# 4ment/physher

Measured on NVIDIA B200. Metric: lnL+gradient throughput (site patterns x tree nodes per second), higher is better.
Workload: dtype f64

## Files before the change

physher_b200/csrc/phb_nuc4.cu:

```cuda
#include "phb_ctx.cuh"

#include <math.h>
#include <stdlib.h>
#include <string.h>

#define NUC4_CHUNK PHBC_WALK_CHUNK
#define NUC4_NT 256
#ifndef NUC4_L2PF
#define NUC4_L2PF 1
#endif

struct Nuc4Params {
	int T, N, C, P, PB, root;
	int n_post, n_pre, nslots, ntiles;
	int include_root_freqs, compat;
	int nbatch, phases;
	long long mats_stride;
	int post_first_tips, pre_first_tips;
	double threshold;
	const uint8_t *tip_codes;
	const double *weights;
	const double *props;
	const phbc_post_op *post_ops;
	const phbc_pre_op *pre_ops;
	const double *post_mats;
	const double *pre_mats;
	double *lower;
	double *gacc;
	double *gstat;
	double *cta_lnl;
	double *pattern_lnl;
	double freqs[4];
	double fq[4];
	double wroot[4];
	double FQ[16];
	double FQ2[16];
	const double *rates;
	double *hacc;
};

__device__ __forceinline__ void matvec_smem(const double *__restrict__ M, const double (&x)[4], double (&y)[4]) {
	const double2 *M2 = reinterpret_cast<const double2 *>(M);
#pragma unroll
	for (int i = 0; i < 4; i++) {
		const double2 a = M2[2 * i], b = M2[2 * i + 1];
		y[i] = fma(a.x, x[0], fma(a.y, x[1], fma(b.x, x[2], b.y * x[3])));
	}
}

__device__ __forceinline__ void tip_message(const double *__restrict__ M, unsigned code, double (&y)[4]) {
	if (__all_sync(0xffffffffu, code < 4u)) {
#pragma unroll
		for (int i = 0; i < 4; i++) y[i] = M[4 * i + code];
	} else {
		double x[4];
#pragma unroll
		for (int j = 0; j < 4; j++) x[j] = (code < 4u ? code == (unsigned)j : ((code >> j) & 1u)) ? 1.0 : 0.0;
		matvec_smem(M, x, y);
		if (code == 4u) y[0] = y[1] = y[2] = y[3] = 1.0;
	}
}

#define NUC4_SLOT_BYTES (2 * NUC4_NT * 16)
#define NUC4_ROW_BYTES (NUC4_NT * 32)

__device__ __forceinline__ void cell_load(const unsigned char *cell, double (&x)[4]) {
	const double2 lo = *reinterpret_cast<const double2 *>(cell);
	const double2 hi = *reinterpret_cast<const double2 *>(cell + NUC4_NT * 16);
	x[0] = lo.x, x[1] = lo.y, x[2] = hi.x, x[3] = hi.y;
}
__device__ __forceinline__ void cell_store(unsigned char *cell, const double (&x)[4]) {
	*reinterpret_cast<double2 *>(cell) = make_double2(x[0], x[1]);
	*reinterpret_cast<double2 *>(cell + NUC4_NT * 16) = make_double2(x[2], x[3]);
}
__device__ __forceinline__ void row_load(const unsigned char *cell, double (&x)[4]) {
	const double2 lo = __ldcs(reinterpret_cast<const double2 *>(cell));
	const double2 hi = __ldcs(reinterpret_cast<const double2 *>(cell + NUC4_NT * 16));
	x[0] = lo.x, x[1] = lo.y, x[2] = hi.x, x[3] = hi.y;
}
__device__ __forceinline__ void row_store(unsigned char *cell, const double (&x)[4]) {
	__stcs(reinterpret_cast<double2 *>(cell), make_double2(x[0], x[1]));
	__stcs(reinterpret_cast<double2 *>(cell + NUC4_NT * 16), make_double2(x[2], x[3]));
}

struct Nuc4Stage {
	uint32_t desc_off, mat_off, code_off, bytes;
};
__host__ __device__ constexpr Nuc4Stage nuc4_stage_layout(int C, int PB) {
	return Nuc4Stage{64u, (uint32_t)(64 + NUC4_CHUNK * 48), (uint32_t)(64 + NUC4_CHUNK * 48 + NUC4_CHUNK * 3 * C * 128),
	                 (uint32_t)((64 + NUC4_CHUNK * 48 + NUC4_CHUNK * 3 * C * 128 + 2 * NUC4_CHUNK * PB + 127) & ~127)};
}

__device__ __forceinline__ double butterfly4(double v0, double v1, double v2, double v3, int lane) {
	const bool h16 = lane & 16, h8 = lane & 8;
	const double r01 = (h16 ? v1 : v0) + __shfl_xor_sync(0xffffffffu, h16 ? v0 : v1, 16);
	const double r23 = (h16 ? v3 : v2) + __shfl_xor_sync(0xffffffffu, h16 ? v2 : v3, 16);
	double r = (h8 ? r23 : r01) + __shfl_xor_sync(0xffffffffu, h8 ? r01 : r23, 8);
	r += __shfl_xor_sync(0xffffffffu, r, 4);
	r += __shfl_xor_sync(0xffffffffu, r, 2);
	r += __shfl_xor_sync(0xffffffffu, r, 1);
	return r;
}
__device__ __forceinline__ double butterfly2(double v0, double v1, int lane) {
	const bool h16 = lane & 16;
	double r = (h16 ? v1 : v0) + __shfl_xor_sync(0xffffffffu, h16 ? v0 : v1, 16);
	r += __shfl_xor_sync(0xffffffffu, r, 8);
	r += __shfl_xor_sync(0xffffffffu, r, 4);
	r += __shfl_xor_sync(0xffffffffu, r, 2);
	r += __shfl_xor_sync(0xffffffffu, r, 1);
	return r;
}

__device__ __forceinline__ void tip_vector(unsigned code, double (&x)[4]) {
#pragma unroll
	for (int j = 0; j < 4; j++) x[j] = (code < 4u ? code == (unsigned)j : (code == 4u || ((code >> j) & 1u))) ? 1.0 : 0.0;
}

template <int PPT>
__device__ __forceinline__ void gstat_add(const double (&t)[PPT][4], const double (&x)[PPT][4], double *row, int lane) {
	double v[16];
#pragma unroll
	for (int i = 0; i < 4; i++)
#pragma unroll
		for (int j = 0; j < 4; j++) {
			double a = t[0][i] * x[0][j];
#pragma unroll
			for (int u = 1; u < PPT; u++) a = fma(t[u][i], x[u][j], a);
			v[4 * i + j] = a;
		}
#pragma unroll
	for (int w = 8, off = 16; w >= 1; w >>= 1, off >>= 1) {
		const bool h = lane & off;
#pragma unroll
		for (int k = 0; k < w; k++) {
			const double keep = h ? v[w + k] : v[k], send = h ? v[k] : v[w + k];
			v[k] = keep + __shfl_xor_sync(0xffffffffu, send, off);
		}
	}
	v[0] += __shfl_xor_sync(0xffffffffu, v[0], 1);
	if (!(lane & 1)) red_add_f64(row + (lane >> 1), v[0]);
}

template <int PPT>
__device__ __forceinline__ void matvec_smem_n(const double *__restrict__ M, const double (&x)[PPT][4], double (&y)[PPT][4]) {
	const double2 *M2 = reinterpret_cast<const double2 *>(M);
#pragma unroll
	for (int i = 0; i < 4; i++) {
		const double2 a = M2[2 * i], b = M2[2 * i + 1];
#pragma unroll
		for (int u = 0; u < PPT; u++) y[u][i] = fma(a.x, x[u][0], fma(a.y, x[u][1], fma(b.x, x[u][2], b.y * x[u][3])));
	}
}

template <int C, bool SCALE, int GRAD, int PPT>
__global__ void __launch_bounds__(NUC4_NT / PPT, GRAD == 3 ? (PPT == 1 ? 1 : 2) : 3) k_nuc4_walk(const Nuc4Params prm) {
	extern __shared__ __align__(128) unsigned char smem_raw[];
	constexpr int PB = NUC4_NT / C;
	constexpr int NTHR = NUC4_NT / PPT;
	constexpr int PBT = PB / PPT;
	static_assert(PBT % 32 == 0 || PPT == 1, "a warp must not mix categories");
	static_assert(GRAD != 3 || !SCALE, "the Hessian walk is unscaled (rescaled evaluations take the resident-partials route)");
	constexpr bool RECOMP = GRAD == 1 && !SCALE;
	const int tid = threadIdx.x, lane = tid & 31, warp = tid >> 5;
	const int c = tid / PBT, pl0 = tid - c * PBT;
	const int cell0 = c * PB + pl0;
	constexpr Nuc4Stage lay = nuc4_stage_layout(C, PB);
	uint64_t *bars = reinterpret_cast<uint64_t *>(smem_raw);
	unsigned char *stage0 = smem_raw;
	unsigned char *slot_cell = stage0 + 2 * lay.bytes + cell0 * 16;
	double *xch = reinterpret_cast<double *>(stage0 + 2 * lay.bytes + (size_t)prm.nslots * NUC4_SLOT_BYTES);
	double *invLw = xch + (SCALE ? (GRAD == 2 ? 5 : 4) : (GRAD == 3 ? 2 : 1)) * C * PB;
	double *sfslot = invLw + PB;
	const uint32_t my_mat = lay.mat_off + c * 128;
	const uint32_t my_code = lay.code_off + pl0;

	if (tid == 0) {
		mbar_init(&bars[0], 1);
		mbar_init(&bars[1], 1);
		asm volatile("fence.mbarrier_init.release.cluster;" ::: "memory");
	}
	__syncthreads();

	uint32_t loads = 0;
	const double prop_c = (C == 1) ? 1.0 : prm.props[c];
	double cta_lnl = 0.0;
	unsigned char *row_cell = GRAD ? reinterpret_cast<unsigned char *>(prm.lower) + (size_t)blockIdx.x * prm.n_post * NUC4_ROW_BYTES + cell0 * 16 : nullptr;
	double *my_gacc = nullptr;
	double *my_gstat = GRAD == 2 ? prm.gstat + ((size_t)blockIdx.x * (NTHR / 32) + warp) * prm.N * 16 : nullptr;
	double *my_hacc = GRAD == 3 ? prm.hacc + ((size_t)blockIdx.x * (NTHR / 32) + warp) * prm.N : nullptr;
	const double rate_c = GRAD == 3 ? prm.rates[c] : 0.0;

	constexpr int PF_LPR = PPT * 2 * 4;
	const int pf_row = (lane / PF_LPR) & 1, pf_q = lane % PF_LPR;
	const bool pf_on = GRAD && lane < 2 * PF_LPR;
	const unsigned char *pf_base = GRAD ? row_cell - lane * 16 + ((pf_q >> 3) * PBT) * 16 + ((pf_q >> 2) & 1) * (NUC4_NT * 16) + (pf_q & 3) * 128 : nullptr;

	const long long nitems = (long long)prm.ntiles * prm.nbatch;
	const bool strided = prm.nbatch == 1;
	const int item0 = strided ? (int)blockIdx.x : (int)(blockIdx.x * nitems / gridDim.x);
	const int item1 = strided ? (int)nitems : (int)((blockIdx.x + 1) * nitems / gridDim.x);
	const int item_step = strided ? (int)gridDim.x : 1;
	const int b_first = strided ? 0 : item0 / prm.ntiles;
	int cur_b = -1;
	auto flush_lnl = [&](int b) {
		if (lane == 0) prm.cta_lnl[((size_t)blockIdx.x * prm.phases + (b - b_first)) * (NTHR / 32) + warp] = (c == 0) ? cta_lnl : 0.0;
	};

	for (int item = item0; item < item1; item += item_step) {
		const int bsmp = item / prm.ntiles, tile = item - bsmp * prm.ntiles;
		if (bsmp != cur_b) {
			if (cur_b >= 0) flush_lnl(cur_b);
			cur_b = bsmp;
			cta_lnl = 0.0;
			if (GRAD) my_gacc = prm.gacc + (((size_t)blockIdx.x * prm.phases + (bsmp - b_first)) * (NTHR / 32) + warp) * prm.N;
		}
		const uint8_t *tile_codes_post = prm.tip_codes + (size_t)tile * prm.T * PB;
		const uint8_t *tile_codes_pre = prm.tip_codes + ((size_t)prm.ntiles + tile) * prm.T * PB;

		double out[PPT][4];
// ... 35 lines not shown
					double sf_in[PPT];
#pragma unroll
					for (int u = 0; u < PPT; u++) sf_in[u] = 0.0;
					if (kind == 0) {
#pragma unroll
						for (int u = 0; u < PPT; u++) {
							tip_message(MA, cds[a_idx * PB + u * PBT], ma[u]);
							tip_message(MB, cds[b_idx * PB + u * PBT], out[u]);
						}
					} else {
						if (SCALE) {
#pragma unroll
							for (int u = 0; u < PPT; u++) sf_in[u] = sf_acc[u];
						}
						if (kind == 1) {
#pragma unroll
							for (int u = 0; u < PPT; u++) tip_message(MA, cds[a_idx * PB + u * PBT], ma[u]);
						} else {
#pragma unroll
							for (int u = 0; u < PPT; u++) {
								cell_load(slot_cell + a_idx * NUC4_SLOT_BYTES + u * PBT * 16, ma[u]);
								if (SCALE) sf_in[u] += sfslot[a_idx * NUC4_NT + cell0 + u * PBT];
							}
						}
					}
#pragma unroll
					for (int u = 0; u < PPT; u++)
#pragma unroll
						for (int i = 0; i < 4; i++) lw[u][i] = ma[u][i] * out[u][i];
					if (SCALE) {
						double *mx = xch + ((first + j) & 1) * C * PB;
#pragma unroll
						for (int u = 0; u < PPT; u++) mx[cell0 + u * PBT] = fmax(fmax(lw[u][0], lw[u][1]), fmax(lw[u][2], lw[u][3]));
						__syncthreads();
#pragma unroll
						for (int u = 0; u < PPT; u++) {
							const int pl = pl0 + u * PBT;
							double m = mx[pl];
							for (int cc = 1; cc < C; cc++) m = fmax(m, mx[cc * PB + pl]);
							double sf = 0.0;
							if (m < prm.threshold) {
#pragma unroll
								for (int i = 0; i < 4; i++) lw[u][i] /= m;
								sf = log(m);
							}
							sf_acc[u] = sf + sf_in[u];
							if (dst_slot >= 0) sfslot[dst_slot * NUC4_NT + cell0 + u * PBT] = sf_acc[u];
						}
					}
					matvec_smem_n<PPT>(MN, lw, out);
#pragma unroll
					for (int u = 0; u < PPT; u++) {
						if (dst_slot >= 0) cell_store(slot_cell + dst_slot * NUC4_SLOT_BYTES + u * PBT * 16, out[u]);
						if (GRAD && keep_row) row_store(row_cell + (size_t)(unsigned)(first + j) * NUC4_ROW_BYTES + u * PBT * 16, out[u]);
					}
				}
				loads++;
				__syncthreads();
			}
		}

		{
#pragma unroll
			for (int u = 0; u < PPT; u++) {
				double site = prm.freqs[0] * out[u][0] + prm.freqs[1] * out[u][1] + prm.freqs[2] * out[u][2] + prm.freqs[3] * out[u][3];
				xch[cell0 + u * PBT] = site * prop_c;
			}
			__syncthreads();
			if (c == 0) {
				double v = 0.0;
#pragma unroll
				for (int u = 0; u < PPT; u++) {
					const int pl = pl0 + u * PBT;
					const int p = tile * PB + pl;
					const bool live = p < prm.P;
					double L = xch[pl];
					for (int cc = 1; cc < C; cc++) L += xch[cc * PB + pl];
					double plk = log(L);
					if (SCALE) plk += sf_acc[u];
					const double w = live ? prm.weights[p] : 0.0;
					if (live && prm.nbatch == 1) prm.pattern_lnl[p] = plk;
					invLw[pl] = w / L;
					if (GRAD == 3) invLw[PB + pl] = 1.0 / L;
					v += live ? plk * w : 0.0;
				}
				v = phb_warp_sum(v);
				if (lane == 0) cta_lnl += v;
			}
			__syncthreads();
		}

		if (GRAD) {
			double sgrad[PPT], wk[PPT], rinv[PPT];
#pragma unroll
			for (int u = 0; u < PPT; u++) {
				const int pl = pl0 + u * PBT;
				const int p = tile * PB + pl;
				sgrad[u] = invLw[pl];
				wk[u] = p < prm.P ? prm.weights[p] : 0.0;
				rinv[u] = GRAD == 3 ? invLw[PB + pl] : 0.0;
			}
			if (GRAD == 2) {
				double r[4];
#pragma unroll
				for (int i = 0; i < 4; i++) {
					r[i] = sgrad[0] * out[0][i];
#pragma unroll
					for (int u = 1; u < PPT; u++) r[i] = fma(sgrad[u], out[u][i], r[i]);
				}
				const double tot = butterfly4(r[0], r[1], r[2], r[3], lane);
				if ((lane & 7) == 0) red_add_f64(my_gstat + (size_t)prm.root * 16 + (((lane >> 4) & 1) | ((lane >> 2) & 2)), tot);
			}
			const int nchunks = (prm.n_pre + NUC4_CHUNK - 1) / NUC4_CHUNK;
			auto issue = [&](int ch, uint32_t ld, int tips) {
				const int first = ch * NUC4_CHUNK;
				const int cnt = min(NUC4_CHUNK, prm.n_pre - first);
				unsigned char *dst = stage0 + (ld & 1) * lay.bytes;
				const uint32_t dbytes = cnt * (uint32_t)sizeof(phbc_pre_op), mbytes = cnt * 3 * C * 128;
				const uint32_t cbytes = (tips & 31) * PB;
				mbar_expect_tx(&bars[ld & 1], dbytes + mbytes + cbytes);
				bulk_g2s(dst + lay.desc_off, prm.pre_ops + first, dbytes, &bars[ld & 1]);
				bulk_g2s(dst + lay.mat_off, prm.pre_mats + (size_t)cur_b * prm.mats_stride + (size_t)first * 3 * C * 16, mbytes, &bars[ld & 1]);
				if (cbytes) bulk_g2s(dst + lay.code_off, tile_codes_pre + (size_t)(tips >> 5) * PB, cbytes, &bars[ld & 1]);
			};
			auto fetch = [&](const phbc_pre_op *d, double (&A)[PPT][4], double (&B)[PPT][4]) {
				const int kind = d->kind;
				const bool b_row = kind != 0 && !(RECOMP && (d->flags & PHBC_PRE_B_RECOMPUTE));
#pragma unroll
				for (int u = 0; u < PPT; u++) {
					if (kind == 2) row_load(row_cell + (size_t)(unsigned)d->a_row * NUC4_ROW_BYTES + u * PBT * 16, A[u]);
					if (b_row) row_load(row_cell + (size_t)(unsigned)d->b_row * NUC4_ROW_BYTES + u * PBT * 16, B[u]);
				}
			};
			constexpr bool ALT = GRAD != 2;
			constexpr bool L2PF = NUC4_L2PF && GRAD != 2;
			auto pre_op = [&](const phbc_pre_op *desc, const unsigned char *mats, const uint8_t *cds, int j, int cnt, bool more_chunks,
			                  double (&xa)[PPT][4], double (&xb)[PPT][4], double (&na_)[PPT][4], double (&nb_)[PPT][4], double (&ureg)[PPT][4],
			                  double &va, double &vb, double &ha, double &hb) {
				const phbc_pre_op *d = desc + j;
				const int kind = d->kind;
				auto prefetch = [&]() {
					if (j + 1 < cnt) {
						fetch(d + 1, na_, nb_);
					} else if (more_chunks) {
						mbar_wait(&bars[(loads + 1) & 1], ((loads + 1) >> 1) & 1);
// ... 221 lines not shown
			};
			if (tid == 0) issue(0, loads, prm.pre_first_tips);
			mbar_wait(&bars[loads & 1], (loads >> 1) & 1);
			static_assert(NUC4_CHUNK % 2 == 0, "the two operand register sets alternate in pairs of ops");
			double xa[PPT][4], xb[PPT][4], ya[PPT][4], yb[PPT][4], ureg[PPT][4];
#pragma unroll
			for (int u = 0; u < PPT; u++)
#pragma unroll
				for (int i = 0; i < 4; i++) xa[u][i] = xb[u][i] = ya[u][i] = yb[u][i] = ureg[u][i] = 0.0;
			fetch(reinterpret_cast<const phbc_pre_op *>(stage0 + (loads & 1) * lay.bytes + lay.desc_off), xa, xb);
			for (int ch = 0; ch < nchunks; ch++) {
				const unsigned char *st = stage0 + (loads & 1) * lay.bytes;
				const phbc_pre_op *desc = reinterpret_cast<const phbc_pre_op *>(st + lay.desc_off);
				if (tid == 0 && ch + 1 < nchunks) issue(ch + 1, loads + 1, desc[0].next_tips);
				const unsigned char *mats = st + my_mat;
				const uint8_t *cds = st + my_code;
				const int first = ch * NUC4_CHUNK;
				const int cnt = min(NUC4_CHUNK, prm.n_pre - first);
				const bool more = ch + 1 < nchunks;
#pragma unroll 1
				for (int j = 0; j < cnt; j += 2) {
					double v0, v1, v2 = 0.0, v3 = 0.0;
					double h0 = 0.0, h1 = 0.0, h2 = 0.0, h3 = 0.0;
					if (ALT) pre_op(desc, mats, cds, j, cnt, more, xa, xb, ya, yb, ureg, v0, v1, h0, h1);
					else pre_op(desc, mats, cds, j, cnt, more, xa, xb, xa, xb, ureg, v0, v1, h0, h1);
					if (j + 1 < cnt) {
						if (ALT) pre_op(desc, mats, cds, j + 1, cnt, more, ya, yb, xa, xb, ureg, v2, v3, h2, h3);
						else pre_op(desc, mats, cds, j + 1, cnt, more, xa, xb, xa, xb, ureg, v2, v3, h2, h3);
						const double r = butterfly4(v0, v1, v2, v3, lane);
						if ((lane & 7) == 0) {
							const phbc_pre_op *d = desc + j + ((lane >> 3) & 1);
							red_add_f64(my_gacc + ((lane & 16) ? d->b_node : d->a_node), r);
						}
						if (GRAD == 3) {
							const double rh = butterfly4(h0, h1, h2, h3, lane);
							if ((lane & 7) == 0) {
								const phbc_pre_op *d = desc + j + ((lane >> 3) & 1);
								red_add_f64(my_hacc + ((lane & 16) ? d->b_node : d->a_node), rh);
							}
						}
					} else {
						const double r = butterfly2(v0, v1, lane);
						if ((lane & 15) == 0) red_add_f64(my_gacc + ((lane & 16) ? desc[j].b_node : desc[j].a_node), r);
						if (GRAD == 3) {
							const double rh = butterfly2(h0, h1, lane);
							if ((lane & 15) == 0) red_add_f64(my_hacc + ((lane & 16) ? desc[j].b_node : desc[j].a_node), rh);
						}
					}
				}
				loads++;
				__syncthreads();
			}
		}
	}
	if (cur_b >= 0) flush_lnl(cur_b);
}

__global__ void k_nuc4_matrices(int T, int C, int root, int n_post, int n_pre, const phbc_post_op *__restrict__ post_ops,
                                const phbc_pre_op *__restrict__ pre_ops, const double *__restrict__ evec,
                                const double *__restrict__ eval, const double *__restrict__ ivec, const double *__restrict__ bl,
                                const double *__restrict__ rates, double *__restrict__ post_mats, double *__restrict__ pre_mats, int N,
                                long long mats_stride) {
	const int e = blockIdx.x * blockDim.x + threadIdx.x;
	const int total = (3 * n_post + 3 * n_pre) * C;
	if (e >= total) return;
	bl += (size_t)blockIdx.y * N;
	post_mats += (size_t)blockIdx.y * mats_stride;
	pre_mats += (size_t)blockIdx.y * mats_stride;
	const int c = e % C;
	const int m = e / C;
	int node, which;
	double *dst;
	if (m < 3 * n_post) {
		const phbc_post_op op = post_ops[m / 3];
		which = m % 3;
		node = which == 0 ? op.node : (which == 1 ? op.a_node : op.b_node);
		dst = post_mats + (size_t)e * 16;
	} else {
		const int mm = m - 3 * n_post;
		const phbc_pre_op op = pre_ops[mm / 3];
		which = mm % 3;
		node = which == 0 ? op.node : (which == 1 ? op.a_node : op.b_node);
		dst = pre_mats + ((size_t)mm * C + c) * 16;
	}
	if (which != 0 && node >= T) return;
	if (node == root) {
		const double diag = m < 3 * n_post ? 1.0 : 0.0;
#pragma unroll
		for (int k = 0; k < 16; k++) dst[k] = (k % 5 == 0) ? diag : 0.0;
		return;
	}
	const double t = bl[node] * rates[c];
	double ex[4];
#pragma unroll
	for (int k = 0; k < 4; k++) ex[k] = exp(eval[k] * t);
#pragma unroll
	for (int i = 0; i < 4; i++)
#pragma unroll
		for (int j = 0; j < 4; j++) {
			double acc = 0.0;
#pragma unroll
			for (int k = 0; k < 4; k++) acc = __dadd_rn(acc, __dmul_rn(__dmul_rn(ivec[k * 4 + j], ex[k]), evec[i * 4 + k]));
			dst[i * 4 + j] = fabs(acc);
		}
}

__global__ void k_nuc4_encode_tips(int T, int P, int PB, int ntiles, int tip_kind, const uint8_t *__restrict__ states,
                                   const double *__restrict__ partials, const int *__restrict__ post_order,
                                   const int *__restrict__ pre_order, uint8_t *__restrict__ codes, int *__restrict__ bad) {
	const size_t per_walk = (size_t)ntiles * T * PB;
	const size_t i = (size_t)blockIdx.x * blockDim.x + threadIdx.x;
	if (i >= 2 * per_walk) return;
	const int walk = i >= per_walk;
	const size_t r = i - walk * per_walk;
	const int pl = (int)(r % PB);
	const int k = (int)((r / PB) % T);
	const int tile = (int)(r / ((size_t)PB * T));
	const int p = tile * PB + pl;
	const int tip = walk ? pre_order[k] : post_order[k];
	unsigned code = 4;
	if (p < P) {
		if (tip_kind == PHBC_TIP_STATES) {
			const unsigned s = states[(size_t)tip * P + p];
			code = s < 4 ? s : 4;
		} else {
			unsigned mask = 0;
			for (int j = 0; j < 4; j++) {
				const double v = partials[((size_t)tip * P + p) * 4 + j];
				if (v == 1.0) mask |= 1u << j;
				else if (v != 0.0) *bad = 1;
			}
			code = __popc(mask) == 1 ? (unsigned)(__ffs(mask) - 1) : (0x10u | mask);
		}
	}
	codes[i] = (uint8_t)code;
}

#define NUC4_FY 16
// ... 85 lines not shown
__global__ void __launch_bounds__(64 * NUC4_GY) k_nuc4_gstat_sum(int N, int C, int nw, int grid, const double *__restrict__ gstat, double *__restrict__ G) {
	__shared__ double red[NUC4_GY][64];
	const int idx = blockIdx.x * 64 + threadIdx.x;
	const bool live = idx < N * C * 16;
	const int e = idx & 15, c = live ? (idx >> 4) % C : 0, n = live ? (idx >> 4) / C : 0;
	const int wpc = nw / C, rows = grid * wpc;
	double s[4] = {0.0, 0.0, 0.0, 0.0};
	if (live) {
		const double *base = gstat + (size_t)n * 16 + e;
		int r = threadIdx.y;
		for (; r + 3 * NUC4_GY < rows; r += 4 * NUC4_GY) {
#pragma unroll
			for (int q = 0; q < 4; q++) {
				const int rr = r + q * NUC4_GY;
				s[q] += base[((size_t)(rr / wpc) * nw + c * wpc + rr % wpc) * N * 16];
			}
		}
		for (; r < rows; r += NUC4_GY) s[0] += base[((size_t)(r / wpc) * nw + c * wpc + r % wpc) * N * 16];
	}
	red[threadIdx.y][threadIdx.x] = (s[0] + s[1]) + (s[2] + s[3]);
	__syncthreads();
	if (threadIdx.y == 0 && live) {
		double tot = 0.0;
#pragma unroll
		for (int k = 0; k < NUC4_GY; k++) tot += red[k][threadIdx.x];
		G[idx] = tot;
	}
}

__global__ void k_nuc4_gstat_contract(int N, int C, int root, int skip, const double *__restrict__ G, const double *__restrict__ M ,
                                      const double *__restrict__ props, double *__restrict__ out) {
	__shared__ double red[256];
	const double *Mk = M + (size_t)blockIdx.x * N * C * 16;
	double s = 0.0;
	for (int nc = threadIdx.x; nc < N * C; nc += blockDim.x) {
		const int n = nc / C, c = nc - n * C;
		if (n == root || n == skip) continue;
		double a = 0.0;
#pragma unroll
		for (int e = 0; e < 16; e++) a = fma(G[(size_t)nc * 16 + e], Mk[(size_t)nc * 16 + e], a);
		s += a * (C == 1 ? 1.0 : props[c]);
	}
	red[threadIdx.x] = s;
	__syncthreads();
	for (int w = blockDim.x / 2; w > 0; w >>= 1) {
		if (threadIdx.x < w) red[threadIdx.x] += red[threadIdx.x + w];
		__syncthreads();
	}
	if (threadIdx.x == 0) out[blockIdx.x] = red[0];
}

static size_t nuc4_smem_bytes(int C, int PB, int nslots, bool scale, int grad) {
	const bool stat = grad == 2, hess = grad == 3 && !scale;
	return 2 * (size_t)nuc4_stage_layout(C, PB).bytes + (size_t)nslots * NUC4_SLOT_BYTES +
	       (size_t)((scale ? (stat ? 5 : 4) : (hess ? 2 : 1)) * C * PB + (hess ? 2 : 1) * PB + (scale ? nslots * NUC4_NT : 0)) * sizeof(double);
}

static int pattern_block(int C) {
	int pb = (NUC4_NT / C) & ~31;
	return pb;
}

bool phbc_nuc4_supported(const phbc_ctx *ctx, const phbc_eval_opts *o) {
	if (ctx->S != 4 || o->explicit_matrices || !ctx->have_eigen) return false;
	if (ctx->C != 1 && ctx->C != 2 && ctx->C != 4 && ctx->C != 8) return false;
	const int PB = pattern_block(ctx->C);
	const int nslots = ctx->post_slots > ctx->pre_slots ? ctx->post_slots : ctx->pre_slots;
	if (nuc4_smem_bytes(ctx->C, PB, nslots, o->scale != 0, o->want_gradient) > ctx->smem_optin) return false;
	return true;
}


static int nuc4_prepare_codes(phbc_ctx *ctx, int *usable);

int phbc_nuc4_evaluate(phbc_ctx *ctx, const phbc_eval_opts *o) {
	PHBC_CHECK(cudaSetDevice(ctx->device));
	const int C = ctx->C, N = ctx->N, T = ctx->T, P = ctx->P;
	const int PB = pattern_block(C);
	const int nslots = ctx->post_slots > ctx->pre_slots ? ctx->post_slots : ctx->pre_slots;
	const size_t smem = nuc4_smem_bytes(C, PB, nslots, o->scale != 0, o->want_gradient);
	const int ntiles = (P + PB - 1) / PB;
	{
		int usable = 0;
		const int prc = nuc4_prepare_codes(ctx, &usable);
		if (prc) return prc;
	}
	ctx->last_family = ctx->nuc4_codes_bad ? 1 : 2;
	if (ctx->nuc4_codes_bad) {
		phbc_eval_opts one = *o;
		one.batch_count = 1;
		for (int b = 0; b < (o->batch_count > 1 ? o->batch_count : 1); b++) {
			one.batch_index = o->batch_index + b;
			const int rc = phbc_generic_evaluate(ctx, &one);
			if (rc) return rc;
		}
		return 0;
	}

	typedef void (*walk_fn)(const Nuc4Params);
	static const walk_fn table[4][2][2] = {
	    {{k_nuc4_walk<1, false, 0, 2>, k_nuc4_walk<1, false, 1, 2>}, {k_nuc4_walk<1, true, 0, 2>, k_nuc4_walk<1, true, 1, 2>}},
	    {{k_nuc4_walk<2, false, 0, 2>, k_nuc4_walk<2, false, 1, 2>}, {k_nuc4_walk<2, true, 0, 2>, k_nuc4_walk<2, true, 1, 2>}},
	    {{k_nuc4_walk<4, false, 0, 2>, k_nuc4_walk<4, false, 1, 2>}, {k_nuc4_walk<4, true, 0, 2>, k_nuc4_walk<4, true, 1, 2>}},
	    {{k_nuc4_walk<8, false, 0, 1>, k_nuc4_walk<8, false, 1, 1>}, {k_nuc4_walk<8, true, 0, 1>, k_nuc4_walk<8, true, 1, 1>}},
	};
	static const walk_fn table_stat[4][2] = {{k_nuc4_walk<1, false, 2, 2>, k_nuc4_walk<1, true, 2, 2>},
	                                         {k_nuc4_walk<2, false, 2, 2>, k_nuc4_walk<2, true, 2, 2>},
	                                         {k_nuc4_walk<4, false, 2, 2>, k_nuc4_walk<4, true, 2, 2>},
	                                         {k_nuc4_walk<8, false, 2, 1>, k_nuc4_walk<8, true, 2, 1>}};
	static const walk_fn table_hess[4] = {k_nuc4_walk<1, false, 3, 2>, k_nuc4_walk<2, false, 3, 2>, k_nuc4_walk<4, false, 3, 2>,
	                                      k_nuc4_walk<8, false, 3, 1>};
	const int ppt = C == 8 ? 1 : 2, nthr = NUC4_NT / ppt;
	const int ci = C == 1 ? 0 : (C == 2 ? 1 : (C == 4 ? 2 : 3));
	const bool want_stat = o->want_gradient == 2, want_hess = o->want_gradient == 3;
	if (want_stat && o->batch_count > 1) {
		snprintf(phbc_errbuf, sizeof(phbc_errbuf), "nuc4 walk: transition statistics need a single-sample evaluation");
		return -1;
	}
	if (want_hess && (o->batch_count > 1 || o->scale)) {
		snprintf(phbc_errbuf, sizeof(phbc_errbuf), "nuc4 walk: the Hessian diagonal needs a single unscaled evaluation");
		return -1;
	}
	walk_fn kern = want_hess ? table_hess[ci] : want_stat ? table_stat[ci][o->scale ? 1 : 0] : table[ci][o->scale ? 1 : 0][o->want_gradient ? 1 : 0];
	ctx->nuc4_G_valid = false;
	PHBC_CHECK(cudaFuncSetAttribute(kern, cudaFuncAttributeMaxDynamicSharedMemorySize, (int)smem));
	int per_sm = 0;
	PHBC_CHECK(cudaOccupancyMaxActiveBlocksPerMultiprocessor(&per_sm, kern, nthr, smem));
	if (per_sm < 1) {
		snprintf(phbc_errbuf, sizeof(phbc_errbuf), "nuc4 walk kernel does not fit on an SM (smem %zu)", smem);
		return -1;
	}
	const int nbatch = o->batch_count > 1 ? o->batch_count : 1;
	const long long nitems = (long long)ntiles * nbatch;
	int grid = per_sm * ctx->num_sms;
	if (grid > nitems) grid = (int)nitems;
	int phases = 1;
	for (int cta = 0; cta < grid; cta++) {
		const long long i0 = cta * nitems / grid, i1 = (cta + 1) * nitems / grid;
		if (i1 > i0) {
			const int ph = (int)((i1 - 1) / ntiles - i0 / ntiles) + 1;
			if (ph > phases) phases = ph;
		}
	}
	const int warps = nthr / 32;
	const long long mats_stride = (long long)(3 * ctx->n_post + 3 * ctx->n_pre) * C * 16;
	const size_t mats_bytes = (size_t)mats_stride * nbatch * sizeof(double);
	if (mats_bytes > ctx->walk_mats_bytes) {
		PHBC_CHECK(cudaStreamSynchronize(ctx->stream));
		if (ctx->d_walk_mats) cudaFree(ctx->d_walk_mats);
		ctx->d_walk_mats = NULL;
		ctx->walk_mats_bytes = 0;
		PHBC_CHECK(cudaMalloc((void **)&ctx->d_walk_mats, mats_bytes));
		ctx->walk_mats_bytes = mats_bytes;
	}
	if (o->want_gradient) {
		const size_t lower_bytes = (size_t)grid * ctx->n_post * NUC4_ROW_BYTES;
		if (lower_bytes > ctx->walk_lower_bytes) {
			PHBC_CHECK(cudaStreamSynchronize(ctx->stream));
			if (ctx->d_walk_lower) cudaFree(ctx->d_walk_lower);
			ctx->d_walk_lower = NULL;
			ctx->walk_lower_bytes = 0;
			PHBC_CHECK(cudaMalloc((void **)&ctx->d_walk_lower, lower_bytes));
			ctx->walk_lower_bytes = lower_bytes;
		}
		const size_t gacc_bytes = (size_t)grid * phases * warps * N * sizeof(double);
		if (gacc_bytes > ctx->walk_gacc_bytes) {
			PHBC_CHECK(cudaStreamSynchronize(ctx->stream));
			if (ctx->d_walk_gacc) cudaFree(ctx->d_walk_gacc);
			ctx->d_walk_gacc = NULL;
			ctx->walk_gacc_bytes = 0;
			PHBC_CHECK(cudaMalloc((void **)&ctx->d_walk_gacc, gacc_bytes));
			ctx->walk_gacc_bytes = gacc_bytes;
		}
		PHBC_CHECK(cudaMemsetAsync(ctx->d_walk_gacc, 0, gacc_bytes, ctx->stream));
	}
	if (want_stat) {
		const size_t gstat_bytes = (size_t)grid * warps * N * 16 * sizeof(double);
		if (gstat_bytes > ctx->walk_gstat_bytes) {
			PHBC_CHECK(cudaStreamSynchronize(ctx->stream));
			if (ctx->d_walk_gstat) cudaFree(ctx->d_walk_gstat);
			ctx->d_walk_gstat = NULL;
			ctx->walk_gstat_bytes = 0;
			PHBC_CHECK(cudaMalloc((void **)&ctx->d_walk_gstat, gstat_bytes));
			ctx->walk_gstat_bytes = gstat_bytes;
		}
		if (!ctx->d_nuc4_G) PHBC_CHECK(cudaMalloc((void **)&ctx->d_nuc4_G, (size_t)N * C * 16 * sizeof(double)));
		PHBC_CHECK(cudaMemsetAsync(ctx->d_walk_gstat, 0, gstat_bytes, ctx->stream));
	}
	if (want_hess) {
		const size_t hacc_bytes = (size_t)grid * warps * N * sizeof(double);
		if (hacc_bytes > ctx->walk_hacc_bytes) {
			PHBC_CHECK(cudaStreamSynchronize(ctx->stream));
			if (ctx->d_walk_hacc) cudaFree(ctx->d_walk_hacc);
			ctx->d_walk_hacc = NULL;
			ctx->walk_hacc_bytes = 0;
			PHBC_CHECK(cudaMalloc((void **)&ctx->d_walk_hacc, hacc_bytes));
			ctx->walk_hacc_bytes = hacc_bytes;
		}
		if (!ctx->d_nuc4_hess) PHBC_CHECK(cudaMalloc((void **)&ctx->d_nuc4_hess, (size_t)N * sizeof(double)));
		PHBC_CHECK(cudaMemsetAsync(ctx->d_walk_hacc, 0, hacc_bytes, ctx->stream));
	}
	if (!ctx->d_nuc4_cta_lnl || ctx->nuc4_grid < grid * phases) {
		PHBC_CHECK(cudaStreamSynchronize(ctx->stream));
		if (ctx->d_nuc4_cta_lnl) cudaFree(ctx->d_nuc4_cta_lnl);
		ctx->d_nuc4_cta_lnl = NULL;
		ctx->nuc4_grid = 0;
		PHBC_CHECK(cudaMalloc((void **)&ctx->d_nuc4_cta_lnl, (size_t)grid * phases * warps * sizeof(double)));
		ctx->nuc4_grid = grid * phases;
	}
	if (nbatch > ctx->cat_grad_cap) {
		PHBC_CHECK(cudaStreamSynchronize(ctx->stream));
		cudaFree(ctx->d_cat_grad);
		ctx->d_cat_grad = NULL;
		ctx->cat_grad_cap = 0;
		PHBC_CHECK(cudaMalloc((void **)&ctx->d_cat_grad, (size_t)nbatch * N * C * sizeof(double)));
		ctx->cat_grad_cap = nbatch;
	}
	double *post_mats = ctx->d_walk_mats;
	double *pre_mats = ctx->d_walk_mats + (size_t)3 * ctx->n_post * C * 16;
	{
		const int total = (3 * ctx->n_post + 3 * ctx->n_pre) * C;
		k_nuc4_matrices<<<dim3((total + 127) / 128, nbatch), 128, 0, ctx->stream>>>(T, C, ctx->root, ctx->n_post, ctx->n_pre, ctx->d_post_ops, ctx->d_pre_ops,
		                                                                          ctx->d_evec, ctx->d_eval, ctx->d_ivec,
		                                                                          ctx->d_bl + (size_t)o->batch_index * N, ctx->d_rates, post_mats, pre_mats,
		                                                                          N, mats_stride);
		ctx->launches++;
	}
	Nuc4Params prm;
	memset(&prm, 0, sizeof(prm));
	prm.T = T, prm.N = N, prm.C = C, prm.P = P, prm.PB = PB, prm.root = ctx->root;
	prm.n_post = ctx->n_post, prm.n_pre = ctx->n_pre, prm.nslots = nslots, prm.ntiles = ntiles;
	prm.include_root_freqs = o->include_root_freqs, prm.compat = o->compat_scaled_gradient;
	prm.nbatch = nbatch, prm.phases = phases, prm.mats_stride = mats_stride;
	prm.post_first_tips = ctx->post_first_tips, prm.pre_first_tips = ctx->pre_first_tips;
	prm.threshold = o->scaling_threshold;
	prm.tip_codes = ctx->d_nuc4_codes;
	prm.weights = ctx->d_weights;
	prm.props = ctx->d_props;
	prm.post_ops = ctx->d_post_ops;
	prm.pre_ops = ctx->d_pre_ops;
	prm.post_mats = post_mats;
	prm.pre_mats = pre_mats;
	prm.lower = ctx->d_walk_lower;
	prm.gacc = ctx->d_walk_gacc;
	prm.gstat = ctx->d_walk_gstat;
	prm.cta_lnl = ctx->d_nuc4_cta_lnl;
	prm.pattern_lnl = ctx->d_pattern_lnl;
	memcpy(prm.freqs, ctx->h_freqs, sizeof(prm.freqs));
	const bool irf = o->include_root_freqs && !want_hess;
	for (int i = 0; i < 4; i++) {
		prm.fq[i] = irf ? 1.0 : ctx->h_freqs[i];
		prm.wroot[i] = irf ? ctx->h_freqs[i] : 1.0;
		for (int j = 0; j < 4; j++) prm.FQ[4 * i + j] = prm.fq[i] * ctx->h_qmat[4 * i + j];
	}
	if (want_hess) {
		for (int i = 0; i < 4; i++)
			for (int j = 0; j < 4; j++) {
				double q2 = 0.0;
				for (int k = 0; k < 4; k++) q2 += ctx->h_qmat[4 * i + k] * ctx->h_qmat[4 * k + j];
				prm.FQ2[4 * i + j] = ctx->h_freqs[i] * q2;
			}
		prm.rates = ctx->d_rates;
		prm.hacc = ctx->d_walk_hacc;
	}
	int trc;
	if ((trc = phbc_time_begin(ctx))) return trc;
	kern<<<grid, nthr, smem, ctx->stream>>>(prm);
	ctx->launches++;
	if ((trc = phbc_time_end(ctx))) return trc;
	double *result = ctx->d_result + (size_t)o->batch_index * (1 + N);
	k_nuc4_finalize<<<dim3((N + 31) / 32, nbatch), dim3(32, NUC4_FY), 0, ctx->stream>>>(N, C, warps, grid, phases, ntiles, nbatch, ctx->root, ctx->d_nuc4_cta_lnl,
	                                                                         ctx->d_walk_gacc, o->want_gradient, ctx->d_props, ctx->d_rates,
	                                                                         ctx->d_cat_grad, result, want_hess ? ctx->d_walk_hacc : NULL,
	                                                                         want_hess ? ctx->d_nuc4_hess : NULL);
	ctx->launches++;
	if (want_stat) {
		k_nuc4_gstat_sum<<<(N * C * 16 + 63) / 64, dim3(64, NUC4_GY), 0, ctx->stream>>>(N, C, warps, grid, ctx->d_walk_gstat, ctx->d_nuc4_G);
		ctx->launches++;
		ctx->nuc4_G_valid = true;
	}
	PHBC_CHECK(cudaGetLastError());
	return 0;
}

static int nuc4_prepare_codes(phbc_ctx *ctx, int *usable) {
	const int C = ctx->C, T = ctx->T, P = ctx->P;
	const int PB = pattern_block(C);
	const int ntiles = (P + PB - 1) / PB;
	if (!ctx->d_nuc4_codes) {
		PHBC_CHECK(cudaMalloc((void **)&ctx->d_nuc4_codes, 2 * (size_t)ntiles * T * PB));
		PHBC_CHECK(cudaMalloc((void **)&ctx->d_nuc4_bad, sizeof(int)));
	}
	if (!ctx->nuc4_codes_valid) {
		const size_t n = 2 * (size_t)ntiles * T * PB;
		PHBC_CHECK(cudaMemsetAsync(ctx->d_nuc4_bad, 0, sizeof(int), ctx->stream));
		k_nuc4_encode_tips<<<(unsigned)((n + 255) / 256), 256, 0, ctx->stream>>>(T, P, PB, ntiles, ctx->tip_kind, ctx->d_tip_states, ctx->d_tip_partials,
		                                                                       ctx->d_post_tip_order, ctx->d_pre_tip_order, ctx->d_nuc4_codes,
		                                                                       ctx->d_nuc4_bad);
		ctx->launches++;
		int bad = 0;
		PHBC_CHECK(cudaMemcpyAsync(&bad, ctx->d_nuc4_bad, sizeof(int), cudaMemcpyDeviceToHost, ctx->stream));
		PHBC_CHECK(cudaStreamSynchronize(ctx->stream));
		ctx->nuc4_codes_bad = bad != 0;
		ctx->nuc4_codes_valid = true;
// ... 112 lines not shown
```

physher_b200/csrc/phb_treelikelihood.c:

```c
#include "../../include/physher_b200.h"
#include "phb_cuda.h"

#include <math.h>
#include <nvtx3/nvToolsExt.h>
#include <stdarg.h>
#include <stdio.h>
#include <stdlib.h>
#include <string.h>

struct phb_tlk {
	int T, N, S, C, P, root;
	int use_tip_states, device;
	int *left, *right, *parent;
	double *bl;
	phbc_ctx *ctx;

	unsigned char *update_nodes;
	int update, update_upper;

	int scale;
	double scaling_threshold;
	int include_root_freqs, compat_scaled_gradient, unrooted, kernels;

	int have_tips, have_weights, have_eigen, have_matrices, have_freqs, have_site, have_bl;
// ... 2 lines not shown
	double lk;
	int prepared_gradient;
	double *gradient;
	size_t gradient_length;
	int gradient_valid;

	phbc_op *lower_ops, *upper_ops;
	phbc_parent_op *parent_ops;
	int *lower_level_off, *upper_level_off, *parent_level_off;
	phbc_post_op *post_ops;
	phbc_pre_op *pre_ops;
	int n_lower_levels, n_upper_levels, post_slots, pre_slots;
	int *post_tip_order, *pre_tip_order, *post_chunk_tip0, *pre_chunk_tip0;
	int post_first_tips, pre_first_tips;
	int have_time_tree;
	int host_exp;
	double *ex_buf;
	size_t ex_cap;
	int sweep_valid;

	int incremental, resident, all_dirty;
	int lower_stale;
	unsigned char *lower_ok, *upper_ok;
	int upper_irf;
	int *upper_op_of;
	phbc_op *sub_ops;
	int *sub_level_off;
	int *path;

	double *h_evec, *h_eval, *h_ivec, *h_freqs, *h_rates, *h_props;
	int has_store;
	double *st_bl, *st_evec, *st_eval, *st_ivec, *st_freqs, *st_rates, *st_props;
	double st_lk;
	int st_update, st_scale, st_have_eigen;
	int eigen_changed, freqs_changed, site_changed, bl_changed;
};

static _Thread_local char g_err[512] = "";

static int fail(int code, const char *fmt, ...) {
	va_list ap;
	va_start(ap, fmt);
	vsnprintf(g_err, sizeof(g_err), fmt, ap);
	va_end(ap);
	return code;
}

static int dev_fail(int rc) { return fail(rc == -3 ? PHB_ENOMEM : (rc == -1 ? PHB_EINVAL : (rc == -4 ? PHB_ESTATE : PHB_ECUDA)), "%s", phbc_last_error()); }

const char *phb_last_error(void) { return g_err; }

int phb_internal_fail(int code, const char *msg) { return fail(code, "%s", msg); }
int phb_device_count(void) { return phbc_device_count(); }
const char *phb_version(void) { return "physher_b200 0.2 (sm_100a; walk kernels r2w, level kernels r2z)"; }


static int is_tip(const phb_tlk *t, int n) { return t->left[n] < 0; }

static int build_level_schedules(phb_tlk *t) {
	const int N = t->N, T = t->T;
	int rc = PHB_OK;
	int *level = (int *)calloc(N, sizeof(int));
	int *depth = (int *)calloc(N, sizeof(int));
	int *order = (int *)malloc(sizeof(int) * N);
	int *stack = (int *)malloc(sizeof(int) * (2 * (size_t)N + 2));
	int *fill = (int *)malloc(sizeof(int) * ((size_t)N + 2));
	if (!level || !depth || !order || !stack || !fill) {
		rc = fail(PHB_ENOMEM, "out of memory");
		goto done;
	}
	int sp = 0, cnt = 0;
	stack[sp++] = t->root;
	while (sp) {
		int n = stack[--sp];
		if (cnt >= N || level[n]) {
			cnt = N + 1;
			break;
		}
		level[n] = 1;
		order[cnt++] = n;
		if (!is_tip(t, n)) {
			depth[t->left[n]] = depth[n] + 1;
			depth[t->right[n]] = depth[n] + 1;
			stack[sp++] = t->right[n];
			stack[sp++] = t->left[n];
		}
	}
	if (cnt != N) {
		rc = fail(PHB_EINVAL, "topology is not a rooted binary tree over %d nodes (visited %d)", N, cnt);
		goto done;
	}
	memset(level, 0, sizeof(int) * N);
	int maxlevel = 0, maxdepth = 0;
	for (int k = N - 1; k >= 0; k--) {
		int n = order[k];
		if (!is_tip(t, n)) {
			int a = level[t->left[n]], b = level[t->right[n]];
			level[n] = 1 + (a > b ? a : b);
		}
		if (level[n] > maxlevel) maxlevel = level[n];
		if (depth[n] > maxdepth) maxdepth = depth[n];
	}
	t->n_lower_levels = maxlevel;
	t->n_upper_levels = maxdepth;
	t->lower_level_off = (int *)calloc(maxlevel + 2, sizeof(int));
	t->lower_ops = (phbc_op *)malloc(sizeof(phbc_op) * (N - T > 0 ? N - T : 1));
	t->upper_level_off = (int *)calloc(maxdepth + 2, sizeof(int));
// ... 1802 lines not shown
```

Measured before the change: 35.72 billion.

## Add DMMA-based adjoint pre-order gradient path for unscaled 4-category walk

For the unscaled first-derivative walk with four rate categories, the pre-order gradient pass is replaced by an adjoint formulation. It uses f64 m8n8k4 tensor-core MMAs to apply combined transition and derivative matrices, and stores post-order rows in an MMA-fragment layout. The matrix kernel precomputes interleaved P and fq-scaled dP/dt matrices for pre-order ops, which doubles the pre-matrix footprint. Occupancy drops to 2 CTAs per SM on this path, and tip gathers and warp butterfly reductions add complexity.

New measurement: 15.42 billion, median of 6. 0.432x the previous value.

```diff
diff --git a/physher_b200/csrc/phb_nuc4.cu b/physher_b200/csrc/phb_nuc4.cu
--- a/physher_b200/csrc/phb_nuc4.cu
+++ b/physher_b200/csrc/phb_nuc4.cu
@@ -1,4 +1,4 @@
-#include "phb_ctx.cuh"
+#include "phb_dmma_common.cuh"
 
 #include <math.h>
 #include <stdlib.h>
@@ -86,10 +86,11 @@
 struct Nuc4Stage {
 	uint32_t desc_off, mat_off, code_off, bytes;
 };
-__host__ __device__ constexpr Nuc4Stage nuc4_stage_layout(int C, int PB) {
-	return Nuc4Stage{64u, (uint32_t)(64 + NUC4_CHUNK * 48), (uint32_t)(64 + NUC4_CHUNK * 48 + NUC4_CHUNK * 3 * C * 128),
-	                 (uint32_t)((64 + NUC4_CHUNK * 48 + NUC4_CHUNK * 3 * C * 128 + 2 * NUC4_CHUNK * PB + 127) & ~127)};
-}
+__host__ __device__ constexpr Nuc4Stage nuc4_stage_layout(int C, int PB, bool adj = false) {
+	return Nuc4Stage{64u, (uint32_t)(64 + NUC4_CHUNK * 48), (uint32_t)(64 + NUC4_CHUNK * 48 + NUC4_CHUNK * 3 * C * (adj ? 256 : 128)),
+	                 (uint32_t)((64 + NUC4_CHUNK * 48 + NUC4_CHUNK * 3 * C * (adj ? 256 : 128) + 2 * NUC4_CHUNK * PB + 127) & ~127)};
+}
+__host__ __device__ constexpr bool nuc4_adjoint(int C, bool scale, int grad) { return grad == 1 && !scale && C == 4; }
 
 __device__ __forceinline__ double butterfly4(double v0, double v1, double v2, double v3, int lane) {
 	const bool h16 = lane & 16, h8 = lane & 8;
@@ -101,6 +102,20 @@
 	r += __shfl_xor_sync(0xffffffffu, r, 1);
 	return r;
 }
+__device__ __forceinline__ double butterfly8(double (&v)[8], int lane) {
+#pragma unroll
+	for (int w = 4, off = 16; w >= 1; w >>= 1, off >>= 1) {
+		const bool h = lane & off;
+#pragma unroll
+		for (int k = 0; k < w; k++) {
+			const double keep = h ? v[w + k] : v[k], send = h ? v[k] : v[w + k];
+			v[k] = keep + __shfl_xor_sync(0xffffffffu, send, off);
+		}
+	}
+	v[0] += __shfl_xor_sync(0xffffffffu, v[0], 2);
+	v[0] += __shfl_xor_sync(0xffffffffu, v[0], 1);
+	return v[0];
+}
 __device__ __forceinline__ double butterfly2(double v0, double v1, int lane) {
 	const bool h16 = lane & 16;
 	double r = (h16 ? v1 : v0) + __shfl_xor_sync(0xffffffffu, h16 ? v0 : v1, 16);
@@ -153,7 +168,7 @@
 }
 
 template <int C, bool SCALE, int GRAD, int PPT>
-__global__ void __launch_bounds__(NUC4_NT / PPT, GRAD == 3 ? (PPT == 1 ? 1 : 2) : 3) k_nuc4_walk(const Nuc4Params prm) {
+__global__ void __launch_bounds__(NUC4_NT / PPT, nuc4_adjoint(C, SCALE, GRAD) ? 2 : (GRAD == 3 ? (PPT == 1 ? 1 : 2) : 3)) k_nuc4_walk(const Nuc4Params prm) {
 	extern __shared__ __align__(128) unsigned char smem_raw[];
 	constexpr int PB = NUC4_NT / C;
 	constexpr int NTHR = NUC4_NT / PPT;
@@ -164,7 +179,9 @@
 	const int tid = threadIdx.x, lane = tid & 31, warp = tid >> 5;
 	const int c = tid / PBT, pl0 = tid - c * PBT;
 	const int cell0 = c * PB + pl0;
-	constexpr Nuc4Stage lay = nuc4_stage_layout(C, PB);
+	constexpr bool ADJ = nuc4_adjoint(C, SCALE, GRAD);
+	static_assert(!ADJ || (PPT == 2 && PBT == 32), "the adjoint pre-order takes 64 patterns of one category per warp");
+	constexpr Nuc4Stage lay = nuc4_stage_layout(C, PB, ADJ);
 	uint64_t *bars = reinterpret_cast<uint64_t *>(smem_raw);
 	unsigned char *stage0 = smem_raw;
 	unsigned char *slot_cell = stage0 + 2 * lay.bytes + cell0 * 16;
@@ -306,7 +323,14 @@
 #pragma unroll
 					for (int u = 0; u < PPT; u++) {
 						if (dst_slot >= 0) cell_store(slot_cell + dst_slot * NUC4_SLOT_BYTES + u * PBT * 16, out[u]);
-						if (GRAD && keep_row) row_store(row_cell + (size_t)(unsigned)(first + j) * NUC4_ROW_BYTES + u * PBT * 16, out[u]);
+						if (GRAD && keep_row && !ADJ) row_store(row_cell + (size_t)(unsigned)(first + j) * NUC4_ROW_BYTES + u * PBT * 16, out[u]);
+						if (ADJ && keep_row) {
+							const int pt = pl0 + u * PBT;
+							unsigned char *row = reinterpret_cast<unsigned char *>(prm.lower) + ((size_t)blockIdx.x * prm.n_post + (unsigned)(first + j)) * NUC4_ROW_BYTES +
+							                     c * 2048 + ((pt & 7) >> 1) * 512 + (pt >> 3) * 64 + (pt & 1) * 8;
+#pragma unroll
+							for (int i = 0; i < 4; i++) __stcs(reinterpret_cast<double *>(row + i * 16), out[u][i]);
+						}
 					}
 				}
 				loads++;
@@ -344,7 +368,7 @@
 			__syncthreads();
 		}
 
-		if (GRAD) {
+		if (GRAD && !ADJ) {
 			double sgrad[PPT], wk[PPT], rinv[PPT];
 #pragma unroll
 			for (int u = 0; u < PPT; u++) {
@@ -672,15 +696,197 @@
 				__syncthreads();
 			}
 		}
+		if constexpr (ADJ) {
+			const int q = lane >> 2, r = lane & 3;
+			const double *sg = invLw + q * 8;
+			const double wr = prm.wroot[r];
+			const unsigned char *lower_cta = reinterpret_cast<const unsigned char *>(prm.lower) + (size_t)blockIdx.x * prm.n_post * NUC4_ROW_BYTES + c * 2048;
+			unsigned char *uslot = stage0 + 2 * lay.bytes + tid * 16;
+			const int nchunks = (prm.n_pre + NUC4_CHUNK - 1) / NUC4_CHUNK;
+			auto issue = [&](int ch, uint32_t ld, int tips) {
+				const int first = ch * NUC4_CHUNK;
+				const int cnt = min(NUC4_CHUNK, prm.n_pre - first);
+				unsigned char *dst = stage0 + (ld & 1) * lay.bytes;
+				const uint32_t dbytes = cnt * (uint32_t)sizeof(phbc_pre_op), mbytes = cnt * 3 * C * 256;
+				const uint32_t cbytes = (tips & 31) * PB;
+				mbar_expect_tx(&bars[ld & 1], dbytes + mbytes + cbytes);
+				bulk_g2s(dst + lay.desc_off, prm.pre_ops + first, dbytes, &bars[ld & 1]);
+				bulk_g2s(dst + lay.mat_off, prm.pre_mats + (size_t)cur_b * prm.mats_stride + (size_t)first * 3 * C * 32, mbytes, &bars[ld & 1]);
+				if (cbytes) bulk_g2s(dst + lay.code_off, tile_codes_pre + (size_t)(tips >> 5) * PB, cbytes, &bars[ld & 1]);
+			};
+			auto fetch = [&](const phbc_pre_op *d, double (&A)[8], double (&B)[8]) {
+				const int kind = d->kind;
+				const bool b_row = kind != 0 && !(d->flags & PHBC_PRE_B_RECOMPUTE);
+				const unsigned char *ra = lower_cta + (size_t)(unsigned)d->a_row * NUC4_ROW_BYTES + lane * 16;
+				const unsigned char *rb = lower_cta + (size_t)(unsigned)d->b_row * NUC4_ROW_BYTES + lane * 16;
+#pragma unroll
+				for (int k = 0; k < 4; k++) {
+					if (kind == 2) {
+						const double2 v = __ldcs(reinterpret_cast<const double2 *>(ra + k * 512));
+						A[2 * k] = v.x, A[2 * k + 1] = v.y;
+					}
+					if (b_row) {
+						const double2 v = __ldcs(reinterpret_cast<const double2 *>(rb + k * 512));
+						B[2 * k] = v.x, B[2 * k + 1] = v.y;
+					}
+				}
+			};
+			auto tip_gather = [&](const unsigned char *img, const uint8_t *codes, double (&M)[8], double (&G)[8], bool want_g) {
+				const uint2 cw = *reinterpret_cast<const uint2 *>(codes);
+				const unsigned char *ir = img + r * 16;
+				const bool fast = __all_sync(0xffffffffu, ((cw.x | cw.y) & 0xfcfcfcfcu) == 0u);
+				const bool sets = !fast && __any_sync(0xffffffffu, ((cw.x | cw.y) & 0x10101010u) != 0u);
+				double rs = 0.0;
+				if (!fast && want_g) {
+#pragma unroll
+					for (int s = 0; s < 4; s++) rs += *reinterpret_cast<const double *>(ir + s * 64 + 8);
+				}
+#pragma unroll
+				for (int t = 0; t < 8; t++) {
+					const unsigned code = ((t < 4 ? cw.x : cw.y) >> (8 * (t & 3))) & 0xffu;
+					double m, g = 0.0;
+					if (want_g) {
+						const double2 v = *reinterpret_cast<const double2 *>(ir + (code & 3u) * 64);
+						m = v.x, g = v.y;
+					} else {
+						m = *reinterpret_cast<const double *>(ir + (code & 3u) * 64);
+					}
+					if (!fast) {
+						if (sets) {
+							double ms = 0.0, gs = 0.0;
+#pragma unroll
+							for (int s = 0; s < 4; s++) {
+								const double f = (code >> s) & 1u ? 1.0 : 0.0;
+								const double2 v = *reinterpret_cast<const double2 *>(ir + s * 64);
+								ms = fma(f, v.x, ms), gs = fma(f, v.y, gs);
+							}
+							m = code >= 0x10u ? ms : m, g = code >= 0x10u ? gs : g;
+						}
+						m = code == 4u ? 1.0 : m, g = code == 4u ? rs : g;
+					}
+					M[t] = m, G[t] = g;
+				}
+			};
+			auto pre_op = [&](const phbc_pre_op *desc, const unsigned char *mats, const uint8_t *cds, int j, int cnt, bool more_chunks,
+			                  double (&xa)[8], double (&xb)[8], double (&na_)[8], double (&nb_)[8], double (&ureg)[8], double &vo, double &va, double &vb) {
+				const phbc_pre_op *d = desc + j;
+				const int kind = d->kind;
+				if (j + 1 < cnt) {
+					fetch(d + 1, na_, nb_);
+				} else if (more_chunks) {
+					mbar_wait(&bars[(loads + 1) & 1], ((loads + 1) >> 1) & 1);
+					fetch(reinterpret_cast<const phbc_pre_op *>(stage0 + ((loads + 1) & 1) * lay.bytes + lay.desc_off), na_, nb_);
+				}
+				if (NUC4_L2PF) {
+					const int rr = reinterpret_cast<const int *>(&d->pf_a_row)[lane >> 4];
+					if (rr >= 0) asm volatile("prefetch.global.L2 [%0];" ::"l"(lower_cta + (size_t)(unsigned)rr * NUC4_ROW_BYTES + (lane & 15) * 128));
+				}
+				const unsigned char *img = mats + j * 3 * C * 256;
+				if (d->flags & PHBC_PRE_B_RECOMPUTE) {
+					const bool same = j + 1 < cnt;
+					const unsigned char *nst = same ? nullptr : stage0 + ((loads + 1) & 1) * lay.bytes;
+					const phbc_pre_op *dn = same ? d + 1 : reinterpret_cast<const phbc_pre_op *>(nst + lay.desc_off);
+					const unsigned char *nimg = same ? img + 3 * C * 256 : nst + lay.mat_off + c * 256;
+					const uint8_t *nc = same ? cds : nst + lay.code_off + q * 8;
+					double ma[8], mb[8], gd[8];
+					tip_gather(nimg + C * 256, nc + dn->a_code * PB, ma, gd, false);
+					tip_gather(nimg + 2 * C * 256, nc + dn->b_code * PB, mb, gd, false);
+					const double bf = reinterpret_cast<const double *>(nimg)[lane];
+#pragma unroll
+					for (int t = 0; t < 8; t++) {
+						double z = 0.0;
+						xb[t] = 0.0;
+						dmma_m8n8k4_nv(xb[t], z, ma[t] * mb[t], bf);
+					}
+				}
+				double ga[8], gb[8];
+				if (kind != 2) tip_gather(img + C * 256, cds + d->a_code * PB, xa, ga, true);
+				if (kind == 0) tip_gather(img + 2 * C * 256, cds + d->b_code * PB, xb, gb, true);
+				double W[8];
+				vo = 0.0;
+				if (d->u_kind == PHBC_W_ROOT) {
+#pragma unroll
+					for (int t = 0; t < 8; t++) W[t] = wr;
+				} else {
+					if (d->u_kind == PHBC_W_SLOT) {
+#pragma unroll
+						for (int k = 0; k < 4; k++) {
+							const double2 v = *reinterpret_cast<const double2 *>(uslot + d->u_slot * NUC4_SLOT_BYTES + k * NTHR * 16);
+							ureg[2 * k] = v.x, ureg[2 * k + 1] = v.y;
+						}
+					}
+					const double bf = reinterpret_cast<const double *>(img)[lane];
+#pragma unroll
+					for (int t = 0; t < 8; t++) {
+						double z = 0.0;
+						W[t] = 0.0;
+						dmma_m8n8k4_nv(W[t], z, ureg[t], bf);
+						vo = fma(sg[t] * z, xa[t] * xb[t], vo);
+					}
+				}
+				va = vb = 0.0;
+				if (kind != 2) {
+#pragma unroll
+					for (int t = 0; t < 8; t++) va = fma(sg[t] * ga[t], W[t] * xb[t], va);
+				}
+				if (kind == 0) {
+#pragma unroll
+					for (int t = 0; t < 8; t++) vb = fma(sg[t] * gb[t], W[t] * xa[t], vb);
+				}
+				if (kind == 2) {
+#pragma unroll
+					for (int k = 0; k < 4; k++)
+						*reinterpret_cast<double2 *>(uslot + d->a_slot * NUC4_SLOT_BYTES + k * NTHR * 16) = make_double2(W[2 * k] * xb[2 * k], W[2 * k + 1] * xb[2 * k + 1]);
+				}
+#pragma unroll
+				for (int t = 0; t < 8; t++) ureg[t] = W[t] * xa[t];
+			};
+			if (tid == 0) issue(0, loads, prm.pre_first_tips);
+			mbar_wait(&bars[loads & 1], (loads >> 1) & 1);
+			static_assert(NUC4_CHUNK % 2 == 0, "the two operand register sets alternate in pairs of ops");
+			double xa[8], xb[8], ya[8], yb[8], ureg[8];
+#pragma unroll
+			for (int t = 0; t < 8; t++) xa[t] = xb[t] = ya[t] = yb[t] = ureg[t] = 0.0;
+			fetch(reinterpret_cast<const phbc_pre_op *>(stage0 + (loads & 1) * lay.bytes + lay.desc_off), xa, xb);
+			for (int ch = 0; ch < nchunks; ch++) {
+				const unsigned char *st = stage0 + (loads & 1) * lay.bytes;
+				const phbc_pre_op *desc = reinterpret_cast<const phbc_pre_op *>(st + lay.desc_off);
+				if (tid == 0 && ch + 1 < nchunks) issue(ch + 1, loads + 1, desc[0].next_tips);
+				const unsigned char *mats = st + lay.mat_off + c * 256;
+				const uint8_t *cds = st + lay.code_off + q * 8;
+				const int first = ch * NUC4_CHUNK;
+				const int cnt = min(NUC4_CHUNK, prm.n_pre - first);
+				const bool more = ch + 1 < nchunks;
+#pragma unroll 1
+				for (int j = 0; j < cnt; j += 2) {
+					double v[8];
+					v[3] = v[4] = v[5] = v[6] = v[7] = 0.0;
+					pre_op(desc, mats, cds, j, cnt, more, xa, xb, ya, yb, ureg, v[0], v[1], v[2]);
+					if (j + 1 < cnt) pre_op(desc, mats, cds, j + 1, cnt, more, ya, yb, xa, xb, ureg, v[4], v[5], v[6]);
+					const double tot = butterfly8(v, lane);
+					const int idx = lane >> 2, w = idx & 3;
+					if ((lane & 3) == 0 && w < 3 && j + (idx >> 2) < cnt) {
+						const phbc_pre_op *d = desc + j + (idx >> 2);
+						const int node = w == 0 ? (d->u_kind == PHBC_W_ROOT ? -1 : d->node) : (w == 1 ? (d->kind != 2 ? d->a_node : -1) : (d->kind == 0 ? d->b_node : -1));
+						if (node >= 0) red_add_f64(my_gacc + node, tot);
+					}
+				}
+				loads++;
+				__syncthreads();
+			}
+		}
 	}
 	if (cur_b >= 0) flush_lnl(cur_b);
 }
 
+struct Nuc4Fq {
+	double v[4];
+};
 __global__ void k_nuc4_matrices(int T, int C, int root, int n_post, int n_pre, const phbc_post_op *__restrict__ post_ops,
                                 const phbc_pre_op *__restrict__ pre_ops, const double *__restrict__ evec,
                                 const double *__restrict__ eval, const double *__restrict__ ivec, const double *__restrict__ bl,
                                 const double *__restrict__ rates, double *__restrict__ post_mats, double *__restrict__ pre_mats, int N,
-                                long long mats_stride) {
+                                long long mats_stride, int adj, Nuc4Fq fq) {
 	const int e = blockIdx.x * blockDim.x + threadIdx.x;
 	const int total = (3 * n_post + 3 * n_pre) * C;
 	if (e >= total) return;
@@ -701,9 +907,48 @@
 		const phbc_pre_op op = pre_ops[mm / 3];
 		which = mm % 3;
 		node = which == 0 ? op.node : (which == 1 ? op.a_node : op.b_node);
-		dst = pre_mats + ((size_t)mm * C + c) * 16;
+		dst = pre_mats + ((size_t)mm * C + c) * (adj ? 32 : 16);
 	}
 	if (which != 0 && node >= T) return;
+	if (adj && m >= 3 * n_post) {
+		if (node == root) {
+#pragma unroll
+			for (int k = 0; k < 32; k++) dst[k] = 0.0;
+			return;
+		}
+		const double t = bl[node] * rates[c];
+		double ex[4], lex[4];
+#pragma unroll
+		for (int k = 0; k < 4; k++) ex[k] = exp(eval[k] * t), lex[k] = eval[k] * ex[k];
+		double Pm[16], Gm[16];
+#pragma unroll
+		for (int i = 0; i < 4; i++)
+#pragma unroll
+			for (int j = 0; j < 4; j++) {
+				double p = 0.0, d = 0.0;
+#pragma unroll
+				for (int k = 0; k < 4; k++) {
+					const double iv = ivec[k * 4 + j], ev = evec[i * 4 + k];
+					p = __dadd_rn(p, __dmul_rn(__dmul_rn(iv, ex[k]), ev));
+					d = __dadd_rn(d, __dmul_rn(__dmul_rn(iv, lex[k]), ev));
+				}
+				Pm[i * 4 + j] = fabs(p);
+				Gm[i * 4 + j] = fq.v[i] * d;
+			}
+		if (which == 0) {
+#pragma unroll
+			for (int l = 0; l < 32; l++) {
+				const int k = l & 3, n = l >> 2;
+				dst[l] = (n & 1) ? Gm[k * 4 + (n >> 1)] : Pm[(n >> 1) * 4 + k];
+			}
+		} else {
+#pragma unroll
+			for (int s = 0; s < 4; s++)
+#pragma unroll
+				for (int r = 0; r < 4; r++) dst[(s * 4 + r) * 2] = Pm[r * 4 + s], dst[(s * 4 + r) * 2 + 1] = Gm[r * 4 + s];
+		}
+		return;
+	}
 	if (node == root) {
 		const double diag = m < 3 * n_post ? 1.0 : 0.0;
 #pragma unroll
@@ -895,7 +1140,7 @@
 
 static size_t nuc4_smem_bytes(int C, int PB, int nslots, bool scale, int grad) {
 	const bool stat = grad == 2, hess = grad == 3 && !scale;
-	return 2 * (size_t)nuc4_stage_layout(C, PB).bytes + (size_t)nslots * NUC4_SLOT_BYTES +
+	return 2 * (size_t)nuc4_stage_layout(C, PB, nuc4_adjoint(C, scale, grad)).bytes + (size_t)nslots * NUC4_SLOT_BYTES +
 	       (size_t)((scale ? (stat ? 5 : 4) : (hess ? 2 : 1)) * C * PB + (hess ? 2 : 1) * PB + (scale ? nslots * NUC4_NT : 0)) * sizeof(double);
 }
 
@@ -986,7 +1231,8 @@
 		}
 	}
 	const int warps = nthr / 32;
-	const long long mats_stride = (long long)(3 * ctx->n_post + 3 * ctx->n_pre) * C * 16;
+	const bool adj = nuc4_adjoint(C, o->scale != 0, o->want_gradient);
+	const long long mats_stride = (long long)(3 * ctx->n_post * 16 + 3 * ctx->n_pre * (adj ? 32 : 16)) * C;
 	const size_t mats_bytes = (size_t)mats_stride * nbatch * sizeof(double);
 	if (mats_bytes > ctx->walk_mats_bytes) {
 		PHBC_CHECK(cudaStreamSynchronize(ctx->stream));
@@ -1061,12 +1307,15 @@
 	}
 	double *post_mats = ctx->d_walk_mats;
 	double *pre_mats = ctx->d_walk_mats + (size_t)3 * ctx->n_post * C * 16;
+	const bool irf = o->include_root_freqs && !want_hess;
+	Nuc4Fq fq;
+	for (int i = 0; i < 4; i++) fq.v[i] = irf ? 1.0 : ctx->h_freqs[i];
 	{
 		const int total = (3 * ctx->n_post + 3 * ctx->n_pre) * C;
 		k_nuc4_matrices<<<dim3((total + 127) / 128, nbatch), 128, 0, ctx->stream>>>(T, C, ctx->root, ctx->n_post, ctx->n_pre, ctx->d_post_ops, ctx->d_pre_ops,
 		                                                                          ctx->d_evec, ctx->d_eval, ctx->d_ivec,
 		                                                                          ctx->d_bl + (size_t)o->batch_index * N, ctx->d_rates, post_mats, pre_mats,
-		                                                                          N, mats_stride);
+		                                                                          N, mats_stride, adj ? 1 : 0, fq);
 		ctx->launches++;
 	}
 	Nuc4Params prm;
@@ -1090,9 +1339,8 @@
 	prm.cta_lnl = ctx->d_nuc4_cta_lnl;
 	prm.pattern_lnl = ctx->d_pattern_lnl;
 	memcpy(prm.freqs, ctx->h_freqs, sizeof(prm.freqs));
-	const bool irf = o->include_root_freqs && !want_hess;
 	for (int i = 0; i < 4; i++) {
-		prm.fq[i] = irf ? 1.0 : ctx->h_freqs[i];
+		prm.fq[i] = fq.v[i];
 		prm.wroot[i] = irf ? ctx->h_freqs[i] : 1.0;
 		for (int j = 0; j < 4; j++) prm.FQ[4 * i + j] = prm.fq[i] * ctx->h_qmat[4 * i + j];
 	}
diff --git a/physher_b200/csrc/phb_treelikelihood.c b/physher_b200/csrc/phb_treelikelihood.c
--- a/physher_b200/csrc/phb_treelikelihood.c
+++ b/physher_b200/csrc/phb_treelikelihood.c
@@ -78,7 +78,7 @@
 
 int phb_internal_fail(int code, const char *msg) { return fail(code, "%s", msg); }
 int phb_device_count(void) { return phbc_device_count(); }
-const char *phb_version(void) { return "physher_b200 0.2 (sm_100a; walk kernels r2w, level kernels r2z)"; }
+const char *phb_version(void) { return "physher_b200 0.2 (sm_100a; walk kernels r4w, level kernels r2z)"; }
 
 
 static int is_tip(const phb_tlk *t, int n) { return t->left[n] < 0; }
```
